# AwesomePeiweiPan/Droid-SLAM_Reserch

Measured on AMD Instinct MI355X. Metric: BA update iters/sec (2000-edge equivalents; 256 keyframes, 48x64), higher is better.
Workload: dtype f32; 1 GPU; 256-keyframe / 2000-edge global BA, 48x64, t0=1, lm=1e-5 ep=1e-2 (BASELINE configs[2]); edges_total=2000, solve=fp64 dense Cholesky on device, chol_failed=False

## Files before the change

### droid-slam_reserch_amd/csrc/ba_kernels.hip

```cpp
#include <hip/hip_runtime.h>
#include <stdint.h>
#include <stdlib.h>

#include "ba_internal.hpp"
#include "se3.hpp"

namespace droid {


__device__ void block_exscan(int* data, int L, int* lds, int* total) {
  const int T = blockDim.x, t = threadIdx.x, lane = t & 63, wave = t >> 6, nw = T >> 6;
  const int per = (L + T - 1) / T;
  const int b = t * per;
  int s = 0;
  for (int k = 0; k < per; k++)
    if (b + k < L) s += data[b + k];
  int incl = s;
#pragma unroll
  for (int off = 1; off < 64; off <<= 1) {
    const int v = __shfl_up(incl, off);
    if (lane >= off) incl += v;
  }
  if (lane == 63) lds[wave] = incl;
  __syncthreads();
// ... 772 lines not shown
            float selfacc[6] = {0.f, 0.f, 0.f, 0.f, 0.f, 0.f};
            const bool self_here = has_self && r0 == 0;
            int ent_base = has_self ? 1 : 0;
            for (int c0 = 0; c0 < nedges; c0 += SLOT_MAXE) {
              const int cnt = min(SLOT_MAXE, nedges - c0);
              if (!resident) {
                __syncthreads();
                load_slot_meta(sm, v, poses, jj, f, x_beg + c0, cnt, ent_base);
                for (int u = 0; u < cnt; u++) ent_base += (sm.ent[u] >= 0) ? 1 : 0;
              }
              for (int x = part; x < cnt; x += 4) {
                const int a = sm.ent[x];
                const bool in_blk = a >= a_beg && a < a_end;
                if (!(in_blk || self_here)) continue;
                float T[12];
#pragma unroll
                for (int n = 0; n < 12; n++) T[n] = sm.T[x][n];
                float eij[6] = {0.f, 0.f, 0.f, 0.f, 0.f, 0.f};
                if (pok) {
                  float wu_raw, wv_raw;
                  const int u = x >> 2;
                  if (resident && u < SF_PF) {
                    wu_raw = cur_w[0];
                    wv_raw = cur_w[1];
#pragma unroll
                    for (int uu = 1; uu < SF_PF; uu++)
                      if (u == uu) {
                        wu_raw = cur_w[2 * uu];
                        wv_raw = cur_w[2 * uu + 1];
                      }
                  } else {
                    const float* wg = weights + (size_t)sm.e[x] * 2 * HW;
                    wu_raw = wg[k];
                    wv_raw = wg[HW + k];
                  }
                  e_row(K, T, sm.flag[x] != 0, ((float)(k % W) - K.cx) / K.fx, ((float)(k / W) - K.cy) / K.fy, disp, wu_raw, wv_raw, eij);
                }
                if (self_here) {
                  float eii[6];
                  adjT_mat(T, T + 9, eij, eii);
#pragma unroll
                  for (int n = 0; n < 6; n++) selfacc[n] -= eii[n];
                }
                if (in_blk) {
#pragma unroll
                  for (int n = 0; n < 6; n++) {
                    const int row = 6 * a + n - r0;
                    if (row >= 0 && row < nrow) buf[row * SF_PITCH + pixl] = eij[n] * sq;
                  }
                }
              }
            }
            if (self_here) {
#pragma unroll
              for (int n = 0; n < 6; n++) SP[(part * 6 + n) * SF_TP + pixl] = selfacc[n];
              __syncthreads();
              for (int n = part; n < 6; n += 4) {
                const float sum = (SP[(0 * 6 + n) * SF_TP + pixl] + SP[(1 * 6 + n) * SF_TP + pixl]) +
                                  (SP[(2 * 6 + n) * SF_TP + pixl] + SP[(3 * 6 + n) * SF_TP + pixl]);
                buf[n * SF_PITCH + pixl] = sum * sq;
              }
              if (ba != bb) __syncthreads();
            }
            const int rows_pad = ((side ? nb : na) + 15) & ~15;
            for (int row = nrow + part; row < rows_pad; row += 4) buf[row * SF_PITCH + pixl] = 0.f;
          }
          if (ba == nblk - 1 && part == 0) {
            EA[(R - ra0) * SF_PITCH + pixl] = cur_wr * sq;
          }
        }
        __syncthreads();
        prefetch(tile + 1);
        const int r = lane & 15, g = lane >> 4;
        const float* Bs = (ba == bb) ? EA : EB;
#pragma unroll
        for (int t = 0; t < SF_MAXT; t++) {
          const int ti = wave + 4 * t;
          if (ti < ntiles) {
            int ta, tb;
            if (ba == bb) {
              ta = 0;
              int rem = ti;
              while (rem > ta) {
                rem -= ta + 1;
                ta++;
              }
              tb = rem;
            } else {
              ta = ti / tb_n;
              tb = ti % tb_n;
            }
            const float* pa = &EA[(16 * ta + r) * SF_PITCH + 4 * g];
            const float* pb = &Bs[(16 * tb + r) * SF_PITCH + 4 * g];
            f32x4 c = (f32x4){0.f, 0.f, 0.f, 0.f};
#pragma unroll
            for (int s4 = 0; s4 < SF_TP; s4 += 16) {
              const f32x4 av = *reinterpret_cast<const f32x4*>(pa + s4);
              const f32x4 bv = *reinterpret_cast<const f32x4*>(pb + s4);
#pragma unroll
              for (int e = 0; e < 4; e++) c = __builtin_amdgcn_mfma_f32_16x16x4f32(av[e], bv[e], c, 0, 0, 0);
            }
#pragma unroll
            for (int x = 0; x < 4; x++) tot[t][x] += (double)c[x];
          }
        }
      }
      {
        const int r = lane & 15, g = lane >> 4;
#pragma unroll
        for (int t = 0; t < SF_MAXT; t++) {
          const int ti = wave + 4 * t;
          if (ti >= ntiles) continue;
          int ta, tb;
          if (ba == bb) {
            ta = 0;
            int rem = ti;
            while (rem > ta) {
              rem -= ta + 1;
              ta++;
            }
            tb = rem;
          } else {
            ta = ti / tb_n;
            tb = ti % tb_n;
          }
#pragma unroll
          for (int x = 0; x < 4; x++) {
            const int li = ra0 + 16 * ta + 4 * g + x;
            const int lj = rb0 + 16 * tb + r;
            if (lj >= R || li > R) continue;
            const double val = -tot[t][x];
            const int gj = 6 * v.ent_pose[e0 + lj / 6] + lj % 6;
            if (li == R) {
              atomicAdd(sys_at(v, v.n, gj), val);
              continue;
            }
            const int gi = 6 * v.ent_pose[e0 + li / 6] + li % 6;
            const bool diag_tile = (ba == bb) && (ta == tb);
            if (diag_tile) {
              if (gi >= gj) atomicAdd(sys_at(v, gi, gj), val);
            } else {
              if (gi > gj) atomicAdd(sys_at(v, gi, gj), val);
              else if (gi < gj) atomicAdd(sys_at(v, gj, gi), val);
              else atomicAdd(sys_at(v, gi, gj), 2.0 * val);
            }
          }
        }
      }
    }
  }
}


constexpr int S2_MAXT = 6;
struct Schur2Meta {
  int e[S2_MAXE];
  int flag[S2_MAXE];
  float T[S2_MAXE][12];
};

__device__ __forceinline__ int s2_swz(int row) { return (((row + 4) >> 3) & 1) << 2; }
__global__ __launch_bounds__(256, 3) void ba_schur2_kernel(BaView v, const float* __restrict__ poses,
                                                           const float* __restrict__ disps,
                                                           const float* __restrict__ intrinsics,
                                                           const float* __restrict__ weights,
                                                           const int64_t* __restrict__ ii,
                                                           const int64_t* __restrict__ jj, int wide, int asm_units) {
  __shared__ __attribute__((aligned(16))) float EB[6 * S2_MAXE * SF_PITCH];
  __shared__ Schur2Meta sm;
  if ((int)blockIdx.x >= v.M) {
    AssembleScratch* sh = reinterpret_cast<AssembleScratch*>(EB);
    const int unit = (((int)blockIdx.x - v.M) * (int)gridDim.y + (int)blockIdx.y) * 4 + (int)(threadIdx.x >> 6);
    if (unit < asm_units) assemble_unit(v, poses, ii, jj, unit, (int)(threadIdx.x & 63), sh[threadIdx.x >> 6]);
    return;
  }
  if ((int)blockIdx.x >= min(v.hdr[HDR_M], v.M)) return;
  const int m = v.order[blockIdx.x];
  const int tid = threadIdx.x, lane = tid & 63, wave = tid >> 6;
  const int HW = v.HW, W = v.W;
  const int x_beg = v.seg_ptr[m], nedges = v.seg_ptr[m + 1] - x_beg;
  if (nedges == 0 || nedges > S2_MAXE) return;
  const int R = 6 * nedges;
  const int ntr = (R + 15) / 16, ntiles = ntr * (ntr + 1) / 2;
  const int f = v.kx[m];
  const Intr K = {intrinsics[0], intrinsics[1], intrinsics[2], intrinsics[3]};
  const int tiles_total = (HW + SF_TP - 1) / SF_TP;
  const int tpw = (tiles_total + gridDim.y - 1) / gridDim.y;
  const int tile_beg = blockIdx.y * tpw, tile_end = min(tiles_total, tile_beg + tpw);
  if (tile_beg >= tile_end) return;
  const int pixl = tid & (SF_TP - 1), part = tid >> 6;
  if (tid < nedges) {
    const int e = v.seg_edge[x_beg + tid];
    const int jx = (int)jj[e];
    const RelMat<float> T = rel_pose_mat<float, true>(poses, f, jx);
    sm.e[tid] = e;
    sm.flag[tid] = (jx == f) ? 1 : 0;
#pragma unroll
    for (int n = 0; n < 9; n++) sm.T[tid][n] = T.R[n];
#pragma unroll
    for (int n = 0; n < 3; n++) sm.T[tid][9 + n] = T.t[n];
  }
  for (int row = R + part; row < 16 * ntr; row += 4) EB[row * SF_PITCH + pixl] = 0.f;
  __syncthreads();

  constexpr int NU = S2_MAXE / 4;
  float pf_q = 0.f, pf_d = 0.f, pf_wr = 0.f, pf_w[2 * NU];
  auto prefetch = [&](int tile) {
    const int k = tile * SF_TP + pixl;
    const bool ok = (tile < tile_end) && (k < HW);
    pf_q = ok ? v.Q[(size_t)m * HW + k] : 0.f;
    pf_d = ok ? disps[(size_t)f * HW + k] : 0.f;
    pf_wr = ok ? v.w[(size_t)m * HW + k] : 0.f;
#pragma unroll
    for (int u = 0; u < NU; u++) {
      const int x = part + 4 * u;
      const bool okx = ok && x < nedges;
      const float* wg = weights + (size_t)(okx ? sm.e[x] : 0) * 2 * HW;
      pf_w[2 * u] = okx ? wg[k] : 0.f;
      pf_w[2 * u + 1] = okx ? wg[HW + k] : 0.f;
    }
  };

  double tot[S2_MAXT][4];
#pragma unroll
  for (int t = 0; t < S2_MAXT; t++)
#pragma unroll
    for (int x = 0; x < 4; x++) tot[t][x] = 0.0;
  float uacc[NU][6];
#pragma unroll
  for (int u = 0; u < NU; u++)
#pragma unroll
    for (int n = 0; n < 6; n++) uacc[u][n] = 0.f;
  int toff_a[S2_MAXT], toff_b[S2_MAXT];
#pragma unroll
  for (int t = 0; t < S2_MAXT; t++) {
    int ta = 0, rem = min(wave + 4 * t, ntiles - 1);
    while (rem > ta) {
      rem -= ta + 1;
      ta++;
    }
    toff_a[t] = (16 * ta + (lane & 15)) * SF_PITCH + ((4 * (lane >> 4)) ^ s2_swz(lane & 15));
    toff_b[t] = (16 * rem + (lane & 15)) * SF_PITCH + ((4 * (lane >> 4)) ^ s2_swz(lane & 15));
  }

  prefetch(tile_beg);
  for (int tile = tile_beg; tile < tile_end; tile++) {
    const int k = tile * SF_TP + pixl;
    const bool pok = k < HW;
    const float sq = sqrtf(pf_q), disp = pf_d, wq = pf_wr * sq;
    float cur_w[2 * NU];
#pragma unroll
    for (int u = 0; u < 2 * NU; u++) cur_w[u] = pf_w[u];
    if (tile > tile_beg) __syncthreads();
    const float X0 = ((float)(k % W) - K.cx) / K.fx, X1 = ((float)(k / W) - K.cy) / K.fy;
#pragma unroll
    for (int u = 0; u < NU; u++) {
      const int x = part + 4 * u;
      if (x < nedges) {
        float eij[6] = {0.f, 0.f, 0.f, 0.f, 0.f, 0.f};
        if (pok && sm.flag[x] == 0) {
          const float* T = sm.T[x];
          const float px = T[0] * X0 + T[1] * X1 + T[2] + disp * T[9];
          const float py = T[3] * X0 + T[4] * X1 + T[5] + disp * T[10];
          const float pz = T[6] * X0 + T[7] * X1 + T[8] + disp * T[11];
          const bool bad = pz < DROID_MIN_DEPTH;
          const float d = bad ? 0.f : 1.0f / pz;
          PixLin L;
          pix_jacobians(K, px, py, d, disp, T[9], T[10], T[11], L);
          const float val = bad ? 0.f : 0.001f * sq;
          const float su = (val * cur_w[2 * u]) * L.Jzu, sv = (val * cur_w[2 * u + 1]) * L.Jzv;
#pragma unroll
          for (int n = 0; n < 6; n++) eij[n] = su * L.Ju[n] + sv * L.Jv[n];
        }
#pragma unroll
        for (int n = 0; n < 6; n++) {
          EB[(6 * x + n) * SF_PITCH + (pixl ^ s2_swz(6 * x + n))] = eij[n];
          uacc[u][n] = fmaf(eij[n], wq, uacc[u][n]);
        }
      }
    }
    __syncthreads();
    prefetch(tile + 1);
#pragma unroll
    for (int t = 0; t < S2_MAXT; t += 2) {
      const bool two = (t + 1 < S2_MAXT) && (wave + 4 * (t + 1) < ntiles);
      if (two) {
        const float* pa0 = &EB[toff_a[t]];
        const float* pb0 = &EB[toff_b[t]];
        const float* pa1 = &EB[toff_a[t + 1 < S2_MAXT ? t + 1 : t]];
        const float* pb1 = &EB[toff_b[t + 1 < S2_MAXT ? t + 1 : t]];
        f32x4 c0 = (f32x4){0.f, 0.f, 0.f, 0.f}, c1 = (f32x4){0.f, 0.f, 0.f, 0.f};
#pragma unroll
        for (int s4 = 0; s4 < SF_TP; s4 += 16) {
          const f32x4 av0 = *reinterpret_cast<const f32x4*>(pa0 + s4), bv0 = *reinterpret_cast<const f32x4*>(pb0 + s4);
          const f32x4 av1 = *reinterpret_cast<const f32x4*>(pa1 + s4), bv1 = *reinterpret_cast<const f32x4*>(pb1 + s4);
#pragma unroll
          for (int e = 0; e < 4; e++) {
            c0 = __builtin_amdgcn_mfma_f32_16x16x4f32(av0[e], bv0[e], c0, 0, 0, 0);
            c1 = __builtin_amdgcn_mfma_f32_16x16x4f32(av1[e], bv1[e], c1, 0, 0, 0);
          }
        }
#pragma unroll
        for (int x = 0; x < 4; x++) {
          tot[t][x] += (double)c0[x];
          tot[t + 1 < S2_MAXT ? t + 1 : t][x] += (double)c1[x];
        }
      } else if (wave + 4 * t < ntiles) {
        const float* pa = &EB[toff_a[t]];
        const float* pb = &EB[toff_b[t]];
        f32x4 c = (f32x4){0.f, 0.f, 0.f, 0.f};
#pragma unroll
        for (int s4 = 0; s4 < SF_TP; s4 += 16) {
          const f32x4 av = *reinterpret_cast<const f32x4*>(pa + s4);
          const f32x4 bv = *reinterpret_cast<const f32x4*>(pb + s4);
#pragma unroll
          for (int e = 0; e < 4; e++) c = __builtin_amdgcn_mfma_f32_16x16x4f32(av[e], bv[e], c, 0, 0, 0);
        }
#pragma unroll
        for (int x = 0; x < 4; x++) tot[t][x] += (double)c[x];
      }
    }
  }
  double* gp = v.Gpart + ((size_t)v.gt_ptr[m] * gridDim.y + (size_t)blockIdx.y * (ntiles + 1)) * 256;
#pragma unroll
  for (int t = 0; t < S2_MAXT; t++) {
    const int ti = wave + 4 * t;
    if (ti < ntiles) {
      double* q = gp + (size_t)ti * 256 + 4 * lane;
      *reinterpret_cast<double2*>(q) = make_double2(tot[t][0], tot[t][1]);
      *reinterpret_cast<double2*>(q + 2) = make_double2(tot[t][2], tot[t][3]);
    }
  }
  __syncthreads();
#pragma unroll
  for (int u = 0; u < NU; u++) {
    const int x = part + 4 * u;
    if (x < nedges) {
#pragma unroll
      for (int n = 0; n < 6; n++) EB[(6 * x + n) * SF_TP + ((pixl + 6 * x + n) & (SF_TP - 1))] = uacc[u][n];
    }
  }
  __syncthreads();
  if (tid < R) {
    double sacc = 0.0;
#pragma unroll 8
    for (int c = 0; c < SF_TP; c++) sacc += (double)EB[tid * SF_TP + ((c + tid) & (SF_TP - 1))];
    gp[(size_t)ntiles * 256 + tid] = sacc;
  }
}

constexpr int S2_GP = 6 * S2_MAXE + 1;
constexpr int S2_MAXC = 8;
__global__ __launch_bounds__(1024) void ba_schur_fold_kernel(BaView v, const float* __restrict__ poses,
                                                             const int64_t* __restrict__ jj, int nsplit) {
  __shared__ double G[(6 * S2_MAXE + 1) * S2_GP];
  __shared__ double As[S2_MAXE][6][6];
  __shared__ double Vs[S2_MAXE][6][6];
  __shared__ double Sss[6][6], us[6];
  __shared__ int s_pose[S2_MAXE];
  if ((int)blockIdx.x >= min(v.hdr[HDR_M], v.M)) return;
  const int m = v.order[blockIdx.x];
  const int tid = threadIdx.x, lane = tid & 63, wave = tid >> 6;
  const int x_beg = v.seg_ptr[m], nedges = v.seg_ptr[m + 1] - x_beg;
  if (nedges == 0 || nedges > S2_MAXE) return;
  const int R = 6 * nedges;
  const int ntr = (R + 15) / 16, ntiles = ntr * (ntr + 1) / 2;
  const int f = v.kx[m];
  const int tiles_total = (v.HW + SF_TP - 1) / SF_TP;
  const int tpw = (tiles_total + nsplit - 1) / nsplit;
  const int nchunk = (tiles_total + tpw - 1) / tpw;
  const int e0 = v.ent_ptr[m];
  const bool has_self = (v.ent_ptr[m + 1] > e0) && (v.ent_row[e0] < v.M);
  const int pf = f - v.t0;
  const double* gp = v.Gpart + (size_t)v.gt_ptr[m] * nsplit * 256;
  const size_t cstride = (size_t)(ntiles + 1) * 256;
  if (wave == 15) {
    if (lane < nedges) {
      const int e = v.seg_edge[x_beg + lane];
      const int jx = (int)jj[e];
      const int pj = jx - v.t0;
      s_pose[lane] = (pj >= 0 && pj < v.P) ? pj : -1;
      const RelMat<double> T = rel_pose_mat<double, true>(poses, f, jx);
#pragma unroll
      for (int kk = 0; kk < 6; kk++) {
        double X[6] = {0.0, 0.0, 0.0, 0.0, 0.0, 0.0}, Y[6];
        X[kk] = 1.0;
        adjT_mat(T.R, T.t, X, Y);
#pragma unroll
        for (int r = 0; r < 6; r++) As[lane][r][kk] = Y[r];
      }
    }
  } else if (wave == 14) {
    for (int o = lane; o < R; o += 64) {
      double sacc = 0.0;
      for (int c = 0; c < nchunk; c++) sacc += gp[(size_t)c * cstride + (size_t)ntiles * 256 + o];
      G[R * S2_GP + o] = sacc;
    }
  } else {
    for (int ti = wave; ti < ntiles; ti += 14) {
      int ta = 0, tb = ti;
      while (tb > ta) {
        tb -= ta + 1;
        ta++;
      }
      double a[4] = {0.0, 0.0, 0.0, 0.0};
      for (int c0 = 0; c0 < nchunk; c0 += S2_MAXC) {
        double2 lo[S2_MAXC], hi[S2_MAXC];
#pragma unroll
        for (int c = 0; c < S2_MAXC; c++) {
          const bool ok = c0 + c < nchunk;
          const double* q = gp + (size_t)(ok ? c0 + c : 0) * cstride + (size_t)ti * 256 + 4 * lane;
          lo[c] = *reinterpret_cast<const double2*>(q);
          hi[c] = *reinterpret_cast<const double2*>(q + 2);
          if (!ok) lo[c] = hi[c] = make_double2(0.0, 0.0);
        }
#pragma unroll
        for (int c = 0; c < S2_MAXC; c++) {
          a[0] += lo[c].x; a[1] += lo[c].y; a[2] += hi[c].x; a[3] += hi[c].y;
        }
      }
      const int r = lane & 15, g = lane >> 4;
#pragma unroll
      for (int x = 0; x < 4; x++) {
        const int li = 16 * ta + 4 * g + x, lj = 16 * tb + r;
        if (li >= R || lj >= R) continue;
        G[li * S2_GP + lj] = a[x];
        if (ta != tb) G[lj * S2_GP + li] = a[x];
      }
    }
  }
  __syncthreads();
  if (has_self) {
    for (int o = tid; o < nedges * 36; o += 1024) {
      const int b = o / 36, r = (o / 6) % 6, c = o % 6;
      double sacc = 0.0;
      for (int e = 0; e < nedges; e++)
#pragma unroll
        for (int kk = 0; kk < 6; kk++) sacc -= As[e][r][kk] * G[(6 * e + kk) * S2_GP + 6 * b + c];
      Vs[b][r][c] = sacc;
    }
    if (tid >= 960 && tid < 966) {
      const int r = tid - 960;
      double sacc = 0.0;
      for (int e = 0; e < nedges; e++)
#pragma unroll
        for (int kk = 0; kk < 6; kk++) sacc -= As[e][r][kk] * G[R * S2_GP + 6 * e + kk];
      us[r] = sacc;
    }
    __syncthreads();
    if (tid < 36) {
      const int r = tid / 6, c = tid % 6;
      double sacc = 0.0;
      for (int b = 0; b < nedges; b++)
#pragma unroll
        for (int kk = 0; kk < 6; kk++) sacc -= Vs[b][r][kk] * As[b][c][kk];
      Sss[r][c] = sacc;
    }
    __syncthreads();
  }
  const int nrow = R + (has_self ? 6 : 0);
  const int n = v.n;
  for (int o = tid; o < nrow * nrow; o += 1024) {
    const int ia = o / nrow, ib = o % nrow;
    const int a = ia / 6, r = ia % 6, b = ib / 6, c = ib % 6;
    const int pa = (a == nedges) ? pf : s_pose[a], pb = (b == nedges) ? pf : s_pose[b];
    if (pa < 0 || pb < 0) continue;
    const int gi = 6 * pa + r, gj = 6 * pb + c;
    if (gi < gj) continue;
    double val;
    if (a < nedges && b < nedges) val = G[ia * S2_GP + ib];
    else if (a == nedges && b == nedges) val = Sss[r][c];
    else if (a == nedges) val = Vs[b][r][c];
    else val = Vs[a][c][r];
    atomicAdd(sys_at(v, gi, gj), -val);
  }
  for (int o = tid; o < nrow; o += 1024) {
    const int a = o / 6, r = o % 6;
    const int pa = (a == nedges) ? pf : s_pose[a];
    if (pa < 0) continue;
    const double val = (a == nedges) ? us[r] : G[R * S2_GP + o];
    atomicAdd(sys_at(v, n, 6 * pa + r), -val);
  }
}

__device__ __forceinline__ void tri_coords(int ti, int& ta, int& tb) {
  int a = (int)((sqrtf(8.0f * (float)ti + 1.0f) - 1.0f) * 0.5f);
  if (a * (a + 1) / 2 > ti) a--;
  if ((a + 1) * (a + 2) / 2 <= ti) a++;
  ta = a;
  tb = ti - a * (a + 1) / 2;
}

constexpr int SY_TPX = 32;
constexpr int SY_T1 = 16 * 17 / 2, SY_T2 = 32 * 33 / 2;

typedef __bf16 bf16x8 __attribute__((ext_vector_type(8)));
typedef __bf16 bf16x2 __attribute__((ext_vector_type(2)));
typedef float f32x2 __attribute__((ext_vector_type(2)));
typedef unsigned u32x4 __attribute__((ext_vector_type(4)));

__device__ __forceinline__ unsigned cvt_pk_bf16(float a, float b) {
  const bf16x2 h = __builtin_convertvector((f32x2){a, b}, bf16x2);
  return __builtin_bit_cast(unsigned, h);
}

__device__ __forceinline__ void split3_bf16(const float (&x)[8], u32x4& p0, u32x4& p1, u32x4& p2) {
#pragma unroll
  for (int e = 0; e < 4; e++) {
    const float xa = x[2 * e], xb = x[2 * e + 1];
    const unsigned h0 = cvt_pk_bf16(xa, xb);
    const float ra = xa - __uint_as_float(h0 << 16), rb = xb - __uint_as_float(h0 & 0xffff0000u);
    const unsigned h1 = cvt_pk_bf16(ra, rb);
    const float sa = ra - __uint_as_float(h1 << 16), sb = rb - __uint_as_float(h1 & 0xffff0000u);
    p0[e] = h0;
    p1[e] = h1;
    p2[e] = cvt_pk_bf16(sa, sb);
  }
}

template <int ROWS, int NWV, int CLS, int NSHARE, bool DBUF, bool LANEMAP>
__global__ __launch_bounds__(64 * NWV) void ba_syrk3_kernel(BaView v) {
  constexpr int NW = NWV, NTH = 64 * NWV, NST = (ROWS / 16 + 1) / 2;
  constexpr int MAXS = ((NST * (NST + 1) / 2 + NSHARE - 1) / NSHARE + NW - 1) / NW;
  constexpr int NR = ((ROWS + 15) & ~15) + 16 + (LANEMAP ? 0 : 4);
  constexpr int MAXT = (4 * ROWS + NTH - 1) / NTH;
  constexpr int PD = DBUF ? 2 : 1;
  __shared__ u32x4 PL[(DBUF ? 2 : 1) * 12 * NR];
  const int count = min(v.hdr[HDR_NC1 + CLS - 1], v.M);
  if (count <= 0) return;
  const int HW = v.HW;
  const int stages_total = HW / SY_TPX;
  const int wgs = (int)(gridDim.x * gridDim.y), wlin = (int)(blockIdx.x + gridDim.x * blockIdx.y);
  const int nrange = max(1, min(min(wgs / count, SY_MAXSPLIT), stages_total));
  if (wlin >= count * nrange) return;
  const int m = v.cls_list[(CLS - 1) * (v.nbuf + 2) + wlin % count];
  const int range = wlin / count;
  const int tid = threadIdx.x, lane = tid & 63;
  const int wave = __builtin_amdgcn_readfirstlane(tid >> 6);
  const int e0 = v.ent_ptr[m], nent = v.ent_ptr[m + 1] - e0;
  const int R = 6 * nent;
  const int spw = (stages_total + nrange - 1) / nrange;
  const int st_beg = range * spw, st_end = min(stages_total, st_beg + spw);
  if (st_beg >= st_end) return;
  const int ntr = (R + 1 + 15) / 16;
  const int nst = (ntr + 1) / 2;
  const int nsup_all = nst * (nst + 1) / 2;
  __shared__ unsigned char s_cost[NST * (NST + 1) / 2];
  __shared__ short s_sorted[NST * (NST + 1) / 2];
  for (int i = tid; i < nsup_all; i += (int)blockDim.x) {
    int sa, sb;
    tri_coords(i, sa, sb);
    const int rows2 = (2 * sa + 1 < ntr) ? 2 : 1;
    s_cost[i] = (unsigned char)(sa == sb ? (rows2 == 2 ? 3 : 1) : 2 * rows2);
  }
  __syncthreads();
  for (int i = tid; i < nsup_all; i += (int)blockDim.x) {
    const int c = s_cost[i];
    int pos = 0;
    for (int o = 0; o < nsup_all; o++) {
      const int co = s_cost[o];
      pos += (co > c || (co == c && o < i)) ? 1 : 0;
    }
    if (pos % NSHARE == (int)blockIdx.z) s_sorted[pos / NSHARE] = (short)i;
  }
  __syncthreads();
  const int nsup = (nsup_all - (int)blockIdx.z + NSHARE - 1) / NSHARE;
  if (nsup <= 0) return;
  int mysup[MAXS];
#pragma unroll
  for (int u = 0; u < MAXS; u++) {
    const int kpos = NW * u + ((u & 1) ? NW - 1 - wave : wave);
    mysup[u] = __builtin_amdgcn_readfirstlane(kpos < nsup ? (int)s_sorted[kpos] : -1);
  }

  const int nrows = R + 1;
  const int sg = LANEMAP ? (lane >> 4) : (tid & 3);
  const float* src[MAXT];
  int sstep[MAXT];
  int dst[MAXT];
  bool needed[MAXT];
#pragma unroll
  for (int it = 0; it < MAXT; it++) {
    const int row = (LANEMAP ? 16 * wave + (lane & 15) : (tid >> 2)) + (NTH / 4) * it;
    const int rr = min(row, nrows - 1);
    src[it] = (rr < R ? v.Ebuf + ebuf_index(e0, R, HW, rr, 0) : v.w + (size_t)m * HW) + 8 * sg;
    sstep[it] = rr < R ? 32 * R : 32;
    dst[it] = sg * NR + (row < nrows ? row : NR - 1);
    needed[it] = (NTH / 4) * it + 16 * wave < nrows;
  }
  const float* qsrc = v.Q + (size_t)m * HW + 8 * sg;
  f32x4 pf[PD][MAXT][2], pq[2];
  auto load_q = [&](int st) {
    const size_t o = (size_t)min(st, st_end - 1) * SY_TPX;
    pq[0] = *reinterpret_cast<const f32x4*>(qsrc + o);
    pq[1] = *reinterpret_cast<const f32x4*>(qsrc + o + 4);
  };
  auto load_stage = [&](int st, int k) {
    const size_t sc = (size_t)min(st, st_end - 1);
#pragma unroll
    for (int it = 0; it < MAXT; it++) {
      const float* g = src[it] + sc * sstep[it];
      pf[k][it][0] = *reinterpret_cast<const f32x4*>(g);
      pf[k][it][1] = *reinterpret_cast<const f32x4*>(g + 4);
    }
  };
  auto store_stage = [&](int k, int buf) {
    float sq[8];
#pragma unroll
    for (int e = 0; e < 8; e++) sq[e] = __builtin_amdgcn_sqrtf(pq[e >> 2][e & 3]);
#pragma unroll
    for (int it = 0; it < MAXT; it++) {
      if (needed[it]) {
        float x[8];
#pragma unroll
        for (int e = 0; e < 8; e++) x[e] = pf[k][it][e >> 2][e & 3] * sq[e];
        u32x4 p0, p1, p2;
        split3_bf16(x, p0, p1, p2);
        u32x4* P = PL + buf * 12 * NR + dst[it];
        P[0] = p0;
        P[4 * NR] = p1;
        P[8 * NR] = p2;
      }
    }
  };

  const int r = lane & 15, g = lane >> 4;
  f32x4 acc[MAXS][4];
#pragma unroll
  for (int u = 0; u < MAXS; u++)
#pragma unroll
    for (int q = 0; q < 4; q++) acc[u][q] = (f32x4){0.f, 0.f, 0.f, 0.f};
  const int offl = g * NR + r;
  int offa[MAXS], offb[MAXS];
  bool upper[MAXS], second[MAXS];
#pragma unroll
  for (int u = 0; u < MAXS; u++) {
    int sa, sb;
    tri_coords(max(mysup[u], 0), sa, sb);
    offa[u] = __builtin_amdgcn_readfirstlane(32 * sa);
    offb[u] = __builtin_amdgcn_readfirstlane(32 * sb);
    upper[u] = (sa != sb);
    second[u] = (2 * sa + 1 < ntr);
  }
  const f32x4 zero4 = {0.f, 0.f, 0.f, 0.f};
  auto mm2 = [&](const bf16x8 (&a)[3], const bf16x8 (&b)[3], f32x4& t, const bf16x8 (&a2)[3], const bf16x8 (&b2)[3], f32x4& t2) {
    f32x4 c = __builtin_amdgcn_mfma_f32_16x16x32_bf16(a[0], b[2], zero4, 0, 0, 0);
    f32x4 c2 = __builtin_amdgcn_mfma_f32_16x16x32_bf16(a2[0], b2[2], zero4, 0, 0, 0);
    c = __builtin_amdgcn_mfma_f32_16x16x32_bf16(a[2], b[0], c, 0, 0, 0);
    c2 = __builtin_amdgcn_mfma_f32_16x16x32_bf16(a2[2], b2[0], c2, 0, 0, 0);
    c = __builtin_amdgcn_mfma_f32_16x16x32_bf16(a[1], b[1], c, 0, 0, 0);
    c2 = __builtin_amdgcn_mfma_f32_16x16x32_bf16(a2[1], b2[1], c2, 0, 0, 0);
    c = __builtin_amdgcn_mfma_f32_16x16x32_bf16(a[0], b[1], c, 0, 0, 0);
    c2 = __builtin_amdgcn_mfma_f32_16x16x32_bf16(a2[0], b2[1], c2, 0, 0, 0);
    c = __builtin_amdgcn_mfma_f32_16x16x32_bf16(a[1], b[0], c, 0, 0, 0);
    c2 = __builtin_amdgcn_mfma_f32_16x16x32_bf16(a2[1], b2[0], c2, 0, 0, 0);
    c = __builtin_amdgcn_mfma_f32_16x16x32_bf16(a[0], b[0], c, 0, 0, 0);
    c2 = __builtin_amdgcn_mfma_f32_16x16x32_bf16(a2[0], b2[0], c2, 0, 0, 0);
    t += c;
    t2 += c2;
  };
  auto mm1 = [&](const bf16x8 (&a)[3], const bf16x8 (&b)[3], f32x4& t) {
    f32x4 c = __builtin_amdgcn_mfma_f32_16x16x32_bf16(a[0], b[2], zero4, 0, 0, 0);
    c = __builtin_amdgcn_mfma_f32_16x16x32_bf16(a[2], b[0], c, 0, 0, 0);
    c = __builtin_amdgcn_mfma_f32_16x16x32_bf16(a[1], b[1], c, 0, 0, 0);
    c = __builtin_amdgcn_mfma_f32_16x16x32_bf16(a[0], b[1], c, 0, 0, 0);
    c = __builtin_amdgcn_mfma_f32_16x16x32_bf16(a[1], b[0], c, 0, 0, 0);
    c = __builtin_amdgcn_mfma_f32_16x16x32_bf16(a[0], b[0], c, 0, 0, 0);
    t += c;
  };
  auto multiply = [&](int buf) {
    const u32x4* P = PL + buf * 12 * NR;
    auto frag = [&](int chunk) { return __builtin_bit_cast(bf16x8, P[chunk]); };
#pragma unroll
    for (int u = 0; u < MAXS; u++) {
      if (mysup[u] >= 0) {
        bf16x8 a0[3], a1[3], b0[3], b1[3];
#pragma unroll
        for (int p = 0; p < 3; p++) {
          a0[p] = frag(offl + offa[u] + 4 * p * NR);
          b0[p] = frag(offl + offb[u] + 4 * p * NR);
        }
        if (second[u]) {
#pragma unroll
          for (int p = 0; p < 3; p++) a1[p] = frag(offl + offa[u] + 16 + 4 * p * NR);
          mm2(a0, b0, acc[u][0], a1, b0, acc[u][2]);
#pragma unroll
          for (int p = 0; p < 3; p++) b1[p] = frag(offl + offb[u] + 16 + 4 * p * NR);
          if (upper[u]) mm2(a0, b1, acc[u][1], a1, b1, acc[u][3]);
          else mm1(a1, b1, acc[u][3]);
        } else if (upper[u]) {
#pragma unroll
          for (int p = 0; p < 3; p++) b1[p] = frag(offl + offb[u] + 16 + 4 * p * NR);
          mm2(a0, b0, acc[u][0], a0, b1, acc[u][1]);
        } else {
          mm1(a0, b0, acc[u][0]);
        }
      }
    }
  };

  auto lds_barrier = [&]() { __syncthreads(); };
  if constexpr (!DBUF) {
    load_q(st_beg);
    load_stage(st_beg, 0);
    for (int st = st_beg; st < st_end; st++) {
      lds_barrier();
      store_stage(0, 0);
      lds_barrier();
      load_q(st + 1);
      load_stage(st + 1, 0);
      multiply(0);
    }
  } else {
    load_q(st_beg);
    load_stage(st_beg, 0);
    load_stage(st_beg + 1, 1);
    store_stage(0, 0);
    load_q(st_beg + 1);
    load_stage(st_beg + 2, 0);
    lds_barrier();
    const bool mul_first = (wave & 1) != 0;
    for (int st = st_beg; st < st_end; st += 2) {
      if (mul_first) multiply(0);
      store_stage(1, 1);
      load_q(st + 2);
      load_stage(st + 3, 1);
      if (!mul_first) multiply(0);
      lds_barrier();
      if (mul_first && st + 1 < st_end) multiply(1);
      store_stage(0, 0);
      load_q(st + 3);
      load_stage(st + 4, 0);
      if (!mul_first && st + 1 < st_end) multiply(1);
      lds_barrier();
    }
  }
  float* part = v.sy_part[CLS - 1] + ((size_t)(wlin % count) * nrange + range) * (size_t)((CLS == 1 ? SY_T1 : SY_T2) * 256);
#pragma unroll
  for (int u = 0; u < MAXS; u++) {
    if (mysup[u] >= 0) {
      int sa, sb;
      tri_coords(mysup[u], sa, sb);
#pragma unroll
      for (int q = 0; q < 4; q++) {
        const int ta = 2 * sa + (q >> 1), tb = 2 * sb + (q & 1);
        if (ta >= ntr || tb > ta) continue;
        *reinterpret_cast<f32x4*>(part + (size_t)(ta * (ta + 1) / 2 + tb) * 256 + 4 * lane) = acc[u][q];
      }
    }
  }
}

__global__ __launch_bounds__(256) void ba_syrk_fold_kernel(BaView v, int wgs1, int wgs2) {
  const int cls = (int)blockIdx.z + 1;
  const int count = min(v.hdr[HDR_NC1 + cls - 1], v.M);
  const int pos = (int)blockIdx.x;
  if (pos >= count) return;
  const int tmax = cls == 1 ? SY_T1 : SY_T2;
  const int stages_total = v.HW / SY_TPX;
  const int nrange = max(1, min(min((cls == 1 ? wgs1 : wgs2) / count, SY_MAXSPLIT), stages_total));
  const int spw = (stages_total + nrange - 1) / nrange;
  const int nused = (stages_total + spw - 1) / spw;
  const int m = v.cls_list[(cls - 1) * (v.nbuf + 2) + pos];
  const int tid = threadIdx.x, lane = tid & 63, wave = tid >> 6;
  const int e0 = v.ent_ptr[m], nent = v.ent_ptr[m + 1] - e0;
  const int R = 6 * nent;
  const int ntr = (R + 1 + 15) / 16, ntiles = ntr * (ntr + 1) / 2;
  __shared__ int s_pose[SLOT_MAXE + 2];
  for (int i = tid; i < nent; i += (int)blockDim.x) s_pose[i] = v.ent_pose[e0 + i];
  __syncthreads();
  const float* part = v.sy_part[cls - 1] + (size_t)pos * nrange * tmax * 256;
  const int r = lane & 15, g = lane >> 4;
  for (int ti = (int)blockIdx.y * 4 + wave; ti < ntiles; ti += 4 * (int)gridDim.y) {
    int ta, tb;
    tri_coords(ti, ta, tb);
    double sum[4] = {0.0, 0.0, 0.0, 0.0};
    for (int rg = 0; rg < nused; rg++) {
      const f32x4 pv = *reinterpret_cast<const f32x4*>(part + ((size_t)rg * tmax + ti) * 256 + 4 * lane);
#pragma unroll
      for (int x = 0; x < 4; x++) sum[x] += (double)pv[x];
    }
    const int lj = 16 * tb + r;
    if (lj >= R) continue;
    const int gj = 6 * s_pose[lj / 6] + lj % 6;
#pragma unroll
    for (int x = 0; x < 4; x++) {
      const int li = 16 * ta + 4 * g + x;
      if (li > R) continue;
      const double val = -sum[x];
      if (li == R) {
        atomicAdd(sys_at(v, v.n, gj), val);
        continue;
      }
      const int gi = 6 * s_pose[li / 6] + li % 6;
      if (ta == tb) {
        if (gi >= gj) atomicAdd(sys_at(v, gi, gj), val);
      } else {
        if (gi > gj) atomicAdd(sys_at(v, gi, gj), val);
        else if (gi < gj) atomicAdd(sys_at(v, gj, gi), val);
        else atomicAdd(sys_at(v, gi, gj), 2.0 * val);
      }
    }
  }
}

constexpr int BSUB_PPT = 1;

__global__ __launch_bounds__(256) void ba_backsub_kernel(
    BaView v, const float* __restrict__ poses, float* __restrict__ disps,
    const float* __restrict__ intrinsics, const float* __restrict__ weights,
    const int64_t* __restrict__ ii, const int64_t* __restrict__ jj, const double* __restrict__ xsol,
    float* __restrict__ dz_out) {
  __shared__ SlotMeta sm;
  __shared__ float dxs[SLOT_MAXE][6];
  if ((int)blockIdx.x >= min(v.hdr[HDR_M], v.M)) return;
  const int m = v.order[blockIdx.x];
  const int HW = v.HW;
  const int f = v.kx[m];
  const Intr K = {intrinsics[0], intrinsics[1], intrinsics[2], intrinsics[3]};
  int kpix[BSUB_PPT];
  float disp[BSUB_PPT], acc[BSUB_PPT];
  float bx0[BSUB_PPT], bx1[BSUB_PPT];
#pragma unroll
  for (int p = 0; p < BSUB_PPT; p++) {
    kpix[p] = (blockIdx.y * BSUB_PPT + p) * 256 + threadIdx.x;
    disp[p] = kpix[p] < HW ? disps[(size_t)f * HW + kpix[p]] : 0.f;
    acc[p] = 0.f;
    const int kk = kpix[p] < HW ? kpix[p] : 0;
    bx0[p] = ((float)(kk % v.W) - K.cx) / K.fx;
    bx1[p] = ((float)(kk / v.W) - K.cy) / K.fy;
  }
  const int pf = f - v.t0;
  const int e0 = v.ent_ptr[m];
  const bool has_self = (v.ent_ptr[m + 1] > e0) && (v.ent_row[e0] < v.M);
  const bool self_on = has_self && pf > 0;
  const bool failed = v.hdr[HDR_CHOL_FAIL] != 0;
  float dxi[6] = {0.f, 0.f, 0.f, 0.f, 0.f, 0.f};
  if (self_on && !failed)
    for (int n = 0; n < 6; n++) dxi[n] = (float)xsol[6 * pf + n];
  const int x_beg = v.seg_ptr[m], nedges = v.seg_ptr[m + 1] - x_beg;
  for (int c0 = 0; c0 < nedges; c0 += SLOT_MAXE) {
    const int cnt = min(SLOT_MAXE, nedges - c0);
    if (c0 > 0) __syncthreads();
    load_slot_meta(sm, v, poses, jj, f, x_beg + c0, cnt, 0);
    if (threadIdx.x < cnt) {
      const int pj = sm.pj[threadIdx.x];
      const bool on = pj > 0 && pj < v.P;
      float c[6];
// ... 227 lines not shown
```

Before: 2002 iters/s.

## Switch schur2 Gram tiles from fp32 MFMA to 3-way split bf16 MFMA

The schur2 kernel now splits each Jacobian value into three bf16 pieces, paired across neighbouring lanes with DPP, and stores them in a swizzled bf16 plane layout in LDS. The tile products then run on 16x16x32 bf16 MFMAs (six products per pair, emulating fp32), replacing the 16x16x4 fp32 MFMAs, which have much lower throughput. Leftover tiles are split across two waves along K, and the partial sums are reduced through LDS before the store. The split-bf16 emulation drops the lowest-order cross terms, so it can differ slightly from true fp32 accuracy, and the extra conversion and shuffle work at write time adds ALU cost.

```diff
diff --git a/droid-slam_reserch_amd/csrc/ba_kernels.hip b/droid-slam_reserch_amd/csrc/ba_kernels.hip
--- a/droid-slam_reserch_amd/csrc/ba_kernels.hip
+++ b/droid-slam_reserch_amd/csrc/ba_kernels.hip
@@ -948,31 +948,89 @@
 }
 
 
-constexpr int S2_MAXT = 6;
+typedef __bf16 bf16x8 __attribute__((ext_vector_type(8)));
+typedef __bf16 bf16x2 __attribute__((ext_vector_type(2)));
+typedef float f32x2 __attribute__((ext_vector_type(2)));
+typedef unsigned u32x4 __attribute__((ext_vector_type(4)));
+
+__device__ __forceinline__ unsigned cvt_pk_bf16(float a, float b) {
+  const bf16x2 h = __builtin_convertvector((f32x2){a, b}, bf16x2);
+  return __builtin_bit_cast(unsigned, h);
+}
+
+__device__ __forceinline__ void split3_pair(float xa, float xb, unsigned& p0, unsigned& p1, unsigned& p2) {
+  const unsigned h0 = cvt_pk_bf16(xa, xb);
+  const float ra = xa - __uint_as_float(h0 << 16), rb = xb - __uint_as_float(h0 & 0xffff0000u);
+  const unsigned h1 = cvt_pk_bf16(ra, rb);
+  const float sa = ra - __uint_as_float(h1 << 16), sb = rb - __uint_as_float(h1 & 0xffff0000u);
+  p0 = h0;
+  p1 = h1;
+  p2 = cvt_pk_bf16(sa, sb);
+}
+
+__device__ __forceinline__ void split3_bf16(const float (&x)[8], u32x4& p0, u32x4& p1, u32x4& p2) {
+#pragma unroll
+  for (int e = 0; e < 4; e++) {
+    unsigned h0, h1, h2;
+    split3_pair(x[2 * e], x[2 * e + 1], h0, h1, h2);
+    p0[e] = h0;
+    p1[e] = h1;
+    p2[e] = h2;
+  }
+}
+
+__device__ __forceinline__ void mm2(const bf16x8 (&a)[3], const bf16x8 (&b)[3], f32x4& d, const bf16x8 (&a2)[3],
+                                    const bf16x8 (&b2)[3], f32x4& d2) {
+  const f32x4 zero4 = {0.f, 0.f, 0.f, 0.f};
+  f32x4 c = __builtin_amdgcn_mfma_f32_16x16x32_bf16(a[0], b[2], zero4, 0, 0, 0);
+  f32x4 c2 = __builtin_amdgcn_mfma_f32_16x16x32_bf16(a2[0], b2[2], zero4, 0, 0, 0);
+  c = __builtin_amdgcn_mfma_f32_16x16x32_bf16(a[2], b[0], c, 0, 0, 0);
+  c2 = __builtin_amdgcn_mfma_f32_16x16x32_bf16(a2[2], b2[0], c2, 0, 0, 0);
+  c = __builtin_amdgcn_mfma_f32_16x16x32_bf16(a[1], b[1], c, 0, 0, 0);
+  c2 = __builtin_amdgcn_mfma_f32_16x16x32_bf16(a2[1], b2[1], c2, 0, 0, 0);
+  c = __builtin_amdgcn_mfma_f32_16x16x32_bf16(a[0], b[1], c, 0, 0, 0);
+  c2 = __builtin_amdgcn_mfma_f32_16x16x32_bf16(a2[0], b2[1], c2, 0, 0, 0);
+  c = __builtin_amdgcn_mfma_f32_16x16x32_bf16(a[1], b[0], c, 0, 0, 0);
+  c2 = __builtin_amdgcn_mfma_f32_16x16x32_bf16(a2[1], b2[0], c2, 0, 0, 0);
+  d = __builtin_amdgcn_mfma_f32_16x16x32_bf16(a[0], b[0], c, 0, 0, 0);
+  d2 = __builtin_amdgcn_mfma_f32_16x16x32_bf16(a2[0], b2[0], c2, 0, 0, 0);
+}
+__device__ __forceinline__ f32x4 mm1(const bf16x8 (&a)[3], const bf16x8 (&b)[3]) {
+  const f32x4 zero4 = {0.f, 0.f, 0.f, 0.f};
+  f32x4 c = __builtin_amdgcn_mfma_f32_16x16x32_bf16(a[0], b[2], zero4, 0, 0, 0);
+  c = __builtin_amdgcn_mfma_f32_16x16x32_bf16(a[2], b[0], c, 0, 0, 0);
+  c = __builtin_amdgcn_mfma_f32_16x16x32_bf16(a[1], b[1], c, 0, 0, 0);
+  c = __builtin_amdgcn_mfma_f32_16x16x32_bf16(a[0], b[1], c, 0, 0, 0);
+  c = __builtin_amdgcn_mfma_f32_16x16x32_bf16(a[1], b[0], c, 0, 0, 0);
+  return __builtin_amdgcn_mfma_f32_16x16x32_bf16(a[0], b[0], c, 0, 0, 0);
+}
+
+constexpr int S2_NR = 6 * S2_MAXE;
+constexpr int S2_MAXS = 6;
 struct Schur2Meta {
   int e[S2_MAXE];
   int flag[S2_MAXE];
   float T[S2_MAXE][12];
 };
 
-__device__ __forceinline__ int s2_swz(int row) { return (((row + 4) >> 3) & 1) << 2; }
 __global__ __launch_bounds__(256, 3) void ba_schur2_kernel(BaView v, const float* __restrict__ poses,
                                                            const float* __restrict__ disps,
                                                            const float* __restrict__ intrinsics,
                                                            const float* __restrict__ weights,
                                                            const int64_t* __restrict__ ii,
                                                            const int64_t* __restrict__ jj, int wide, int asm_units) {
-  __shared__ __attribute__((aligned(16))) float EB[6 * S2_MAXE * SF_PITCH];
+  __shared__ u32x4 PL[2 * 12 * S2_NR];
   __shared__ Schur2Meta sm;
   if ((int)blockIdx.x >= v.M) {
-    AssembleScratch* sh = reinterpret_cast<AssembleScratch*>(EB);
+    AssembleScratch* sh = reinterpret_cast<AssembleScratch*>(PL);
     const int unit = (((int)blockIdx.x - v.M) * (int)gridDim.y + (int)blockIdx.y) * 4 + (int)(threadIdx.x >> 6);
     if (unit < asm_units) assemble_unit(v, poses, ii, jj, unit, (int)(threadIdx.x & 63), sh[threadIdx.x >> 6]);
     return;
   }
   if ((int)blockIdx.x >= min(v.hdr[HDR_M], v.M)) return;
   const int m = v.order[blockIdx.x];
-  const int tid = threadIdx.x, lane = tid & 63, wave = tid >> 6;
+  const int tid = threadIdx.x, lane = tid & 63;
+  const int wave = __builtin_amdgcn_readfirstlane(tid >> 6);
   const int HW = v.HW, W = v.W;
   const int x_beg = v.seg_ptr[m], nedges = v.seg_ptr[m + 1] - x_beg;
   if (nedges == 0 || nedges > S2_MAXE) return;
@@ -996,7 +1054,13 @@
 #pragma unroll
     for (int n = 0; n < 3; n++) sm.T[tid][9 + n] = T.t[n];
   }
-  for (int row = R + part; row < 16 * ntr; row += 4) EB[row * SF_PITCH + pixl] = 0.f;
+  {
+    const int nz = 16 * ntr - R;
+    for (int i = tid; i < 24 * nz; i += 256) {
+      const int pg = i / nz, row = R + i % nz;
+      PL[pg * S2_NR + (row ^ (2 * (pg & 3)))] = (u32x4){0u, 0u, 0u, 0u};
+    }
+  }
   __syncthreads();
 
   constexpr int NU = S2_MAXE / 4;
@@ -1017,9 +1081,13 @@
     }
   };
 
-  double tot[S2_MAXT][4];
-#pragma unroll
-  for (int t = 0; t < S2_MAXT; t++)
+  const int F = ntiles & ~3, rtl = ntiles & 3;
+  const int nf = F / 4;
+  const int nh = (wave < 2 * rtl ? 1 : 0) + (wave + 4 < 2 * rtl ? 1 : 0);
+  const int hks = wave & 1;
+  double tot[S2_MAXS][4];
+#pragma unroll
+  for (int t = 0; t < S2_MAXS; t++)
 #pragma unroll
     for (int x = 0; x < 4; x++) tot[t][x] = 0.0;
   float uacc[NU][6];
@@ -1027,16 +1095,20 @@
   for (int u = 0; u < NU; u++)
 #pragma unroll
     for (int n = 0; n < 6; n++) uacc[u][n] = 0.f;
-  int toff_a[S2_MAXT], toff_b[S2_MAXT];
-#pragma unroll
-  for (int t = 0; t < S2_MAXT; t++) {
-    int ta = 0, rem = min(wave + 4 * t, ntiles - 1);
+  const int r16 = lane & 15, g = lane >> 4;
+  const int offl = g * S2_NR + (r16 ^ (2 * g));
+  int sa[S2_MAXS], sb[S2_MAXS], stile[S2_MAXS];
+#pragma unroll
+  for (int t = 0; t < S2_MAXS; t++) {
+    const int ti = t < nf ? wave + 4 * t : F + (wave + 4 * (t - nf)) / 2;
+    int ta = 0, rem = min(ti, ntiles - 1);
     while (rem > ta) {
       rem -= ta + 1;
       ta++;
     }
-    toff_a[t] = (16 * ta + (lane & 15)) * SF_PITCH + ((4 * (lane >> 4)) ^ s2_swz(lane & 15));
-    toff_b[t] = (16 * rem + (lane & 15)) * SF_PITCH + ((4 * (lane >> 4)) ^ s2_swz(lane & 15));
+    stile[t] = ti;
+    sa[t] = 16 * ta;
+    sb[t] = 16 * rem;
   }
 
   prefetch(tile_beg);
@@ -1049,6 +1121,10 @@
     for (int u = 0; u < 2 * NU; u++) cur_w[u] = pf_w[u];
     if (tile > tile_beg) __syncthreads();
     const float X0 = ((float)(k % W) - K.cx) / K.fx, X1 = ((float)(k / W) - K.cy) / K.fy;
+    const bool odd = pixl & 1;
+    const int pg = (pixl >> 3) & 3;
+    const int wbase = 4 * ((pixl >> 5) * 12 + pg) * S2_NR + ((pixl & 7) >> 1);
+    unsigned* PW = reinterpret_cast<unsigned*>(PL);
 #pragma unroll
     for (int u = 0; u < NU; u++) {
       const int x = part + 4 * u;
@@ -1069,64 +1145,72 @@
           for (int n = 0; n < 6; n++) eij[n] = su * L.Ju[n] + sv * L.Jv[n];
         }
 #pragma unroll
-        for (int n = 0; n < 6; n++) {
-          EB[(6 * x + n) * SF_PITCH + (pixl ^ s2_swz(6 * x + n))] = eij[n];
-          uacc[u][n] = fmaf(eij[n], wq, uacc[u][n]);
+        for (int n = 0; n < 6; n++) uacc[u][n] = fmaf(eij[n], wq, uacc[u][n]);
+#pragma unroll
+        for (int i = 0; i < 3; i++) {
+          const float keep = odd ? eij[2 * i + 1] : eij[2 * i];
+          const float send = odd ? eij[2 * i] : eij[2 * i + 1];
+          const float recv = __int_as_float(__builtin_amdgcn_update_dpp(0, __float_as_int(send), 0xB1, 0xF, 0xF, false));
+          unsigned h0, h1, h2;
+          split3_pair(odd ? recv : keep, odd ? keep : recv, h0, h1, h2);
+          const int row = 6 * x + 2 * i + (odd ? 1 : 0);
+          const int a = wbase + 4 * (row ^ (2 * pg));
+          PW[a] = h0;
+          PW[a + 4 * 4 * S2_NR] = h1;
+          PW[a + 8 * 4 * S2_NR] = h2;
         }
       }
     }
     __syncthreads();
     prefetch(tile + 1);
 #pragma unroll
-    for (int t = 0; t < S2_MAXT; t += 2) {
-      const bool two = (t + 1 < S2_MAXT) && (wave + 4 * (t + 1) < ntiles);
-      if (two) {
-        const float* pa0 = &EB[toff_a[t]];
-        const float* pb0 = &EB[toff_b[t]];
-        const float* pa1 = &EB[toff_a[t + 1 < S2_MAXT ? t + 1 : t]];
-        const float* pb1 = &EB[toff_b[t + 1 < S2_MAXT ? t + 1 : t]];
-        f32x4 c0 = (f32x4){0.f, 0.f, 0.f, 0.f}, c1 = (f32x4){0.f, 0.f, 0.f, 0.f};
-#pragma unroll
-        for (int s4 = 0; s4 < SF_TP; s4 += 16) {
-          const f32x4 av0 = *reinterpret_cast<const f32x4*>(pa0 + s4), bv0 = *reinterpret_cast<const f32x4*>(pb0 + s4);
-          const f32x4 av1 = *reinterpret_cast<const f32x4*>(pa1 + s4), bv1 = *reinterpret_cast<const f32x4*>(pb1 + s4);
-#pragma unroll
-          for (int e = 0; e < 4; e++) {
-            c0 = __builtin_amdgcn_mfma_f32_16x16x4f32(av0[e], bv0[e], c0, 0, 0, 0);
-            c1 = __builtin_amdgcn_mfma_f32_16x16x4f32(av1[e], bv1[e], c1, 0, 0, 0);
+    for (int ks = 0; ks < 2; ks++) {
+      const int nact = nf + (ks == hks ? nh : 0);
+      const u32x4* P = PL + ks * 12 * S2_NR + offl;
+      auto frag = [&](int row16, int plane) { return __builtin_bit_cast(bf16x8, P[plane * 4 * S2_NR + row16]); };
+#pragma unroll
+      for (int t = 0; t < S2_MAXS; t += 2) {
+        if (t + 1 < S2_MAXS && t + 1 < nact) {
+          bf16x8 a0[3], b0[3], a1[3], b1[3];
+#pragma unroll
+          for (int pl = 0; pl < 3; pl++) {
+            a0[pl] = frag(sa[t], pl);
+            b0[pl] = frag(sb[t], pl);
+            a1[pl] = frag(sa[t + 1 < S2_MAXS ? t + 1 : t], pl);
+            b1[pl] = frag(sb[t + 1 < S2_MAXS ? t + 1 : t], pl);
           }
+          f32x4 c0, c1;
+          mm2(a0, b0, c0, a1, b1, c1);
+#pragma unroll
+          for (int x = 0; x < 4; x++) {
+            tot[t][x] += (double)c0[x];
+            tot[t + 1 < S2_MAXS ? t + 1 : t][x] += (double)c1[x];
+          }
+        } else if (t < nact) {
+          bf16x8 a0[3], b0[3];
+#pragma unroll
+          for (int pl = 0; pl < 3; pl++) {
+            a0[pl] = frag(sa[t], pl);
+            b0[pl] = frag(sb[t], pl);
+          }
+          const f32x4 c0 = mm1(a0, b0);
+#pragma unroll
+          for (int x = 0; x < 4; x++) tot[t][x] += (double)c0[x];
         }
-#pragma unroll
-        for (int x = 0; x < 4; x++) {
-          tot[t][x] += (double)c0[x];
-          tot[t + 1 < S2_MAXT ? t + 1 : t][x] += (double)c1[x];
-        }
-      } else if (wave + 4 * t < ntiles) {
-        const float* pa = &EB[toff_a[t]];
-        const float* pb = &EB[toff_b[t]];
-        f32x4 c = (f32x4){0.f, 0.f, 0.f, 0.f};
-#pragma unroll
-        for (int s4 = 0; s4 < SF_TP; s4 += 16) {
-          const f32x4 av = *reinterpret_cast<const f32x4*>(pa + s4);
-          const f32x4 bv = *reinterpret_cast<const f32x4*>(pb + s4);
-#pragma unroll
-          for (int e = 0; e < 4; e++) c = __builtin_amdgcn_mfma_f32_16x16x4f32(av[e], bv[e], c, 0, 0, 0);
-        }
-#pragma unroll
-        for (int x = 0; x < 4; x++) tot[t][x] += (double)c[x];
       }
     }
   }
   double* gp = v.Gpart + ((size_t)v.gt_ptr[m] * gridDim.y + (size_t)blockIdx.y * (ntiles + 1)) * 256;
-#pragma unroll
-  for (int t = 0; t < S2_MAXT; t++) {
-    const int ti = wave + 4 * t;
-    if (ti < ntiles) {
-      double* q = gp + (size_t)ti * 256 + 4 * lane;
-      *reinterpret_cast<double2*>(q) = make_double2(tot[t][0], tot[t][1]);
-      *reinterpret_cast<double2*>(q + 2) = make_double2(tot[t][2], tot[t][3]);
-    }
-  }
+  auto store_tile = [&](int ti, const double (&q4)[4]) {
+    double* q = gp + (size_t)ti * 256 + 4 * lane;
+    *reinterpret_cast<double2*>(q) = make_double2(q4[0], q4[1]);
+    *reinterpret_cast<double2*>(q + 2) = make_double2(q4[2], q4[3]);
+  };
+#pragma unroll
+  for (int t = 0; t < S2_MAXS; t++)
+    if (t < nf) store_tile(stile[t], tot[t]);
+  float* EB = reinterpret_cast<float*>(PL);
+  double* HB = reinterpret_cast<double*>(PL) + 3 * 1024;
   __syncthreads();
 #pragma unroll
   for (int u = 0; u < NU; u++) {
@@ -1136,7 +1220,24 @@
       for (int n = 0; n < 6; n++) EB[(6 * x + n) * SF_TP + ((pixl + 6 * x + n) & (SF_TP - 1))] = uacc[u][n];
     }
   }
-  __syncthreads();
+  if (hks == 1) {
+#pragma unroll
+    for (int t = 0; t < S2_MAXS; t++)
+      if (t >= nf && t < nf + nh)
+#pragma unroll
+        for (int x = 0; x < 4; x++) HB[((wave >> 1) * 2 + t - nf) * 256 + x * 64 + lane] = tot[t][x];
+  }
+  __syncthreads();
+  if (hks == 0) {
+#pragma unroll
+    for (int t = 0; t < S2_MAXS; t++)
+      if (t >= nf && t < nf + nh) {
+        double q4[4];
+#pragma unroll
+        for (int x = 0; x < 4; x++) q4[x] = tot[t][x] + HB[((wave >> 1) * 2 + t - nf) * 256 + x * 64 + lane];
+        store_tile(stile[t], q4);
+      }
+  }
   if (tid < R) {
     double sacc = 0.0;
 #pragma unroll 8
@@ -1289,30 +1390,6 @@
 
 constexpr int SY_TPX = 32;
 constexpr int SY_T1 = 16 * 17 / 2, SY_T2 = 32 * 33 / 2;
-
-typedef __bf16 bf16x8 __attribute__((ext_vector_type(8)));
-typedef __bf16 bf16x2 __attribute__((ext_vector_type(2)));
-typedef float f32x2 __attribute__((ext_vector_type(2)));
-typedef unsigned u32x4 __attribute__((ext_vector_type(4)));
-
-__device__ __forceinline__ unsigned cvt_pk_bf16(float a, float b) {
-  const bf16x2 h = __builtin_convertvector((f32x2){a, b}, bf16x2);
-  return __builtin_bit_cast(unsigned, h);
-}
-
-__device__ __forceinline__ void split3_bf16(const float (&x)[8], u32x4& p0, u32x4& p1, u32x4& p2) {
-#pragma unroll
-  for (int e = 0; e < 4; e++) {
-    const float xa = x[2 * e], xb = x[2 * e + 1];
-    const unsigned h0 = cvt_pk_bf16(xa, xb);
-    const float ra = xa - __uint_as_float(h0 << 16), rb = xb - __uint_as_float(h0 & 0xffff0000u);
-    const unsigned h1 = cvt_pk_bf16(ra, rb);
-    const float sa = ra - __uint_as_float(h1 << 16), sb = rb - __uint_as_float(h1 & 0xffff0000u);
-    p0[e] = h0;
-    p1[e] = h1;
-    p2[e] = cvt_pk_bf16(sa, sb);
-  }
-}
 
 template <int ROWS, int NWV, int CLS, int NSHARE, bool DBUF, bool LANEMAP>
 __global__ __launch_bounds__(64 * NWV) void ba_syrk3_kernel(BaView v) {
@@ -1438,32 +1515,6 @@
     upper[u] = (sa != sb);
     second[u] = (2 * sa + 1 < ntr);
   }
-  const f32x4 zero4 = {0.f, 0.f, 0.f, 0.f};
-  auto mm2 = [&](const bf16x8 (&a)[3], const bf16x8 (&b)[3], f32x4& t, const bf16x8 (&a2)[3], const bf16x8 (&b2)[3], f32x4& t2) {
-    f32x4 c = __builtin_amdgcn_mfma_f32_16x16x32_bf16(a[0], b[2], zero4, 0, 0, 0);
-    f32x4 c2 = __builtin_amdgcn_mfma_f32_16x16x32_bf16(a2[0], b2[2], zero4, 0, 0, 0);
-    c = __builtin_amdgcn_mfma_f32_16x16x32_bf16(a[2], b[0], c, 0, 0, 0);
-    c2 = __builtin_amdgcn_mfma_f32_16x16x32_bf16(a2[2], b2[0], c2, 0, 0, 0);
-    c = __builtin_amdgcn_mfma_f32_16x16x32_bf16(a[1], b[1], c, 0, 0, 0);
-    c2 = __builtin_amdgcn_mfma_f32_16x16x32_bf16(a2[1], b2[1], c2, 0, 0, 0);
-    c = __builtin_amdgcn_mfma_f32_16x16x32_bf16(a[0], b[1], c, 0, 0, 0);
-    c2 = __builtin_amdgcn_mfma_f32_16x16x32_bf16(a2[0], b2[1], c2, 0, 0, 0);
-    c = __builtin_amdgcn_mfma_f32_16x16x32_bf16(a[1], b[0], c, 0, 0, 0);
-    c2 = __builtin_amdgcn_mfma_f32_16x16x32_bf16(a2[1], b2[0], c2, 0, 0, 0);
-    c = __builtin_amdgcn_mfma_f32_16x16x32_bf16(a[0], b[0], c, 0, 0, 0);
-    c2 = __builtin_amdgcn_mfma_f32_16x16x32_bf16(a2[0], b2[0], c2, 0, 0, 0);
-    t += c;
-    t2 += c2;
-  };
-  auto mm1 = [&](const bf16x8 (&a)[3], const bf16x8 (&b)[3], f32x4& t) {
-    f32x4 c = __builtin_amdgcn_mfma_f32_16x16x32_bf16(a[0], b[2], zero4, 0, 0, 0);
-    c = __builtin_amdgcn_mfma_f32_16x16x32_bf16(a[2], b[0], c, 0, 0, 0);
-    c = __builtin_amdgcn_mfma_f32_16x16x32_bf16(a[1], b[1], c, 0, 0, 0);
-    c = __builtin_amdgcn_mfma_f32_16x16x32_bf16(a[0], b[1], c, 0, 0, 0);
-    c = __builtin_amdgcn_mfma_f32_16x16x32_bf16(a[1], b[0], c, 0, 0, 0);
-    c = __builtin_amdgcn_mfma_f32_16x16x32_bf16(a[0], b[0], c, 0, 0, 0);
-    t += c;
-  };
   auto multiply = [&](int buf) {
     const u32x4* P = PL + buf * 12 * NR;
     auto frag = [&](int chunk) { return __builtin_bit_cast(bf16x8, P[chunk]); };
@@ -1476,20 +1527,30 @@
           a0[p] = frag(offl + offa[u] + 4 * p * NR);
           b0[p] = frag(offl + offb[u] + 4 * p * NR);
         }
+        f32x4 c, c2;
         if (second[u]) {
 #pragma unroll
           for (int p = 0; p < 3; p++) a1[p] = frag(offl + offa[u] + 16 + 4 * p * NR);
-          mm2(a0, b0, acc[u][0], a1, b0, acc[u][2]);
+          mm2(a0, b0, c, a1, b0, c2);
+          acc[u][0] += c;
+          acc[u][2] += c2;
 #pragma unroll
           for (int p = 0; p < 3; p++) b1[p] = frag(offl + offb[u] + 16 + 4 * p * NR);
-          if (upper[u]) mm2(a0, b1, acc[u][1], a1, b1, acc[u][3]);
-          else mm1(a1, b1, acc[u][3]);
+          if (upper[u]) {
+            mm2(a0, b1, c, a1, b1, c2);
+            acc[u][1] += c;
+            acc[u][3] += c2;
+          } else {
+            acc[u][3] += mm1(a1, b1);
+          }
         } else if (upper[u]) {
 #pragma unroll
           for (int p = 0; p < 3; p++) b1[p] = frag(offl + offb[u] + 16 + 4 * p * NR);
-          mm2(a0, b0, acc[u][0], a0, b1, acc[u][1]);
+          mm2(a0, b0, c, a0, b1, c2);
+          acc[u][0] += c;
+          acc[u][1] += c2;
         } else {
-          mm1(a0, b0, acc[u][0]);
+          acc[u][0] += mm1(a0, b0);
         }
       }
     }
```

Result: no change. 2009 iters/s, median of 6 (+0.3%).
